# AIBluefisher/DAGSfM

Hardware: AMD Instinct MI355X
Metric: verified image-pairs/sec (+ RANSAC hypotheses/sec) at 4096 feats/image (higher is better)
Workload: dtype u8 matching (int8 MFMA) + f64 verification

## Files before the change

### dagsfm_amd/csrc/match_kernels.hip

```cpp
#include <hip/hip_runtime.h>
#include <stdint.h>

#include <type_traits>

#include "kernels.h"

typedef int v4i __attribute__((ext_vector_type(4)));
typedef int v16i __attribute__((ext_vector_type(16)));

template <int B, int E, typename F>
__device__ __forceinline__ void static_for(F&& f) {
  if constexpr (B < E) {
    f(std::integral_constant<int, B>());
    static_for<B + 1, E>(f);
  }
}

__global__ __launch_bounds__(256) void k0_prepare(const uint8_t* __restrict__ in_u8,
                                                  int8_t* __restrict__ out_s8,
                                                  int32_t* __restrict__ rterm,
                                                  uint64_t n_rows) {
  const uint64_t gid = (uint64_t)blockIdx.x * blockDim.x + threadIdx.x;
  const uint64_t row = gid >> 3;
  const uint32_t chunk = (uint32_t)gid & 7u;
  if (row >= n_rows) return;
  const uint4 v = reinterpret_cast<const uint4*>(in_u8)[row * 8 + chunk];
  uint32_t w[4] = {v.x, v.y, v.z, v.w};
  int32_t sum = 0;
#pragma unroll
  for (int k = 0; k < 4; ++k) {
    sum += (int32_t)((w[k] & 0xffu) + ((w[k] >> 8) & 0xffu) + ((w[k] >> 16) & 0xffu) + (w[k] >> 24));
    w[k] ^= 0x80808080u;
  }
  uint4 o;
  o.x = w[0]; o.y = w[1]; o.z = w[2]; o.w = w[3];
  reinterpret_cast<uint4*>(out_s8)[row * 8 + chunk] = o;
  sum += __shfl_xor(sum, 1);
  sum += __shfl_xor(sum, 2);
  sum += __shfl_xor(sum, 4);
  if (chunk == 0) rterm[row] = 128 * (sum - 16384);
}

template <int Q>
__device__ __forceinline__ void k1_epilogue_quarter(const v16i& a, int& best, int& second, int& t, int& btile, int tile) {
  if constexpr (Q == 0) {
    asm volatile(
        "v_max3_i32 %[t], %[a0], %[a1], %[a2]\n\t"
        "v_max3_i32 %[t], %[t], %[a3], %[a4]\n\t"
        "v_max3_i32 %[t], %[t], %[a5], %[a6]"
        : [t] "=&v"(t)
        : [a0] "v"(a[0]), [a1] "v"(a[1]), [a2] "v"(a[2]), [a3] "v"(a[3]), [a4] "v"(a[4]), [a5] "v"(a[5]), [a6] "v"(a[6]));
  } else if constexpr (Q == 1) {
    asm volatile(
        "v_max3_i32 %[t], %[t], %[a0], %[a1]\n\t"
        "v_max3_i32 %[t], %[t], %[a2], %[a3]\n\t"
        "v_max3_i32 %[t], %[t], %[a4], %[a5]"
        : [t] "+v"(t)
        : [a0] "v"(a[7]), [a1] "v"(a[8]), [a2] "v"(a[9]), [a3] "v"(a[10]), [a4] "v"(a[11]), [a5] "v"(a[12]));
  } else if constexpr (Q == 2) {
    asm volatile(
        "v_max3_i32 %[t], %[t], %[a0], %[a1]\n\t"
        "v_max3_i32 %[t], %[t], %[a2], %[s]\n\t"
        "v_min_i32 %[s], %[t], %[b]"
        : [t] "+v"(t), [s] "+v"(second)
        : [b] "v"(best), [a0] "v"(a[13]), [a1] "v"(a[14]), [a2] "v"(a[15]));
  } else {
    asm volatile(
        "v_cmp_gt_i32 vcc, %[t], %[b]\n\t"
        "v_cndmask_b32 %[bt], %[bt], %[tile], vcc\n\t"
        "v_max_i32 %[b], %[t], %[b]"
        : [b] "+v"(best), [bt] "+v"(btile)
        : [t] "v"(t), [tile] "v"(tile)
        : "vcc");
  }
}

#ifndef K1_LDS_DMA
#define K1_LDS_DMA 0
#endif
__device__ __forceinline__ int lds_off(int col, int chunk) {
  return col * 128 + ((chunk ^ ((col >> 1) & 7)) << 4);
}

template <bool GATHER>
__global__ __launch_bounds__(256, 2) void k1_best_rows(const K1Params p) {
  const uint32_t d = p.order ? p.order[blockIdx.x] : blockIdx.x;
  const uint32_t rb = blockIdx.y;
  const uint2 ab = p.dpairs[d];
  const uint32_t a_rows = GATHER ? p.e_cnt[d] : p.img_rows[ab.x];
  if (rb * 512u >= a_rows) return;
  const uint32_t b_cols = p.img_rows[ab.y];
  const uint32_t a_row0 = (GATHER ? 0u : p.img_row0[ab.x]) + rb * 512u;
  const uint32_t b_row0 = p.img_row0[ab.y];

  const int tid = threadIdx.x;
  const int lane = tid & 63;
  const int wave = tid >> 6;
  const int l31 = lane & 31;
  const int half = lane >> 5;
  const bool active = rb * 512u + (uint32_t)wave * 128u < a_rows;

  __shared__ __attribute__((aligned(16))) int8_t sB[2][64 * 128];
  __shared__ __attribute__((aligned(16))) int sC[2][64];

  v4i afrag[4][4];
  int rterm_i[4];
  bool valid[4];
  {
    const uint2* ent = GATHER ? p.entries + p.e_off[d] : nullptr;
    const uint32_t img0 = GATHER ? p.img_row0[ab.x] : 0u;
#pragma unroll
    for (int rt = 0; rt < 4; ++rt) {
      const uint32_t r = a_row0 + wave * 128 + rt * 32 + l31;
      valid[rt] = GATHER ? (r < a_rows) : active;
      uint32_t grow = r;
      if (GATHER) grow = valid[rt] ? img0 + ent[r].y : 0u;
      const int8_t* arow = p.desc + (size_t)grow * 128;
#pragma unroll
      for (int ks = 0; ks < 4; ++ks) {
        const v4i z = {0, 0, 0, 0};
        afrag[rt][ks] = valid[rt] ? *reinterpret_cast<const v4i*>(arow + ks * 32 + half * 16) : z;
      }
      rterm_i[rt] = valid[rt] ? p.rterm[grow] : 0;
    }
  }
  int best[4], second[4], btile[4];
#pragma unroll
  for (int rt = 0; rt < 4; ++rt) {
    best[rt] = -rterm_i[rt];
    second[rt] = -rterm_i[rt];
    btile[rt] = 0;
  }

  const int8_t* bimg = p.desc + (size_t)b_row0 * 128;
  const int32_t* rt_b = p.rterm + b_row0;
  const uint32_t nsteps = b_cols >> 6;

  int cstage = 0;
#if K1_LDS_DMA
  const int wave_u = __builtin_amdgcn_readfirstlane(wave);
  int src_off[2];
#pragma unroll
  for (int u = 0; u < 2; ++u) {
    const int L = tid + 256 * u;
    src_off[u] = ((L & ~7) | ((L & 7) ^ ((L >> 4) & 7))) * 16;
  }
  auto stage_tile = [&](const int8_t* src, int buf) {
#pragma unroll
    for (int u = 0; u < 2; ++u)
      __builtin_amdgcn_global_load_lds((const __attribute__((address_space(1))) void*)(src + src_off[u]),
                                       (__attribute__((address_space(3))) void*)(&sB[buf][(wave_u * 64 + 256 * u) * 16]), 16, 0, 0);
  };
  stage_tile(bimg, 0);
  cstage = rt_b[tid & 63];
  if (tid < 64) sC[0][tid] = cstage + (1 << 21);
  __syncthreads();
#else
  v4i stage[2];
#pragma unroll
  for (int u = 0; u < 2; ++u) stage[u] = *reinterpret_cast<const v4i*>(bimg + (size_t)(tid + 256 * u) * 16);
  cstage = rt_b[tid & 63];
#pragma unroll
  for (int u = 0; u < 2; ++u) {
    const int q = tid + 256 * u;
    *reinterpret_cast<v4i*>(&sB[0][lds_off(q >> 3, q & 7)]) = stage[u];
  }
  if (tid < 64) sC[0][tid] = cstage + (1 << 21);
  __syncthreads();
#endif
  asm volatile("s_waitcnt vmcnt(0)" ::: "memory");

  for (uint32_t s = 0; s < nsteps; ++s) {
    const int cur = s & 1;
    const bool more = (s + 1) < nsteps;
    if (more) {
      const int8_t* src = bimg + (size_t)(s + 1) * 64 * 128;
#if K1_LDS_DMA
      stage_tile(src, cur ^ 1);
#else
#pragma unroll
      for (int u = 0; u < 2; ++u) stage[u] = *reinterpret_cast<const v4i*>(src + (size_t)(tid + 256 * u) * 16);
#endif
      cstage = rt_b[(s + 1) * 64 + (tid & 63)];
    }
    if (active) {
      v4i bf0[4], bf1[4];
#pragma unroll
      for (int ks = 0; ks < 4; ++ks) {
        bf0[ks] = *reinterpret_cast<const v4i*>(&sB[cur][lds_off(l31, ks * 2 + half)]);
        bf1[ks] = *reinterpret_cast<const v4i*>(&sB[cur][lds_off(32 + l31, ks * 2 + half)]);
      }
      v16i ci0, ci1;
#pragma unroll
      for (int q = 0; q < 4; ++q) {
        const v4i c0 = *reinterpret_cast<const v4i*>(&sC[cur][8 * q + 4 * half]);
        const v4i c1 = *reinterpret_cast<const v4i*>(&sC[cur][32 + 8 * q + 4 * half]);
#pragma unroll
        for (int e = 0; e < 4; ++e) {
          ci0[4 * q + e] = c0[e];
          ci1[4 * q + e] = c1[e];
        }
      }
      v16i acc[3];
      int tmax;
      int tile_v[2];
      asm volatile("v_mov_b32 %0, %2\n\tv_mov_b32 %1, %3" : "=&v"(tile_v[0]), "=v"(tile_v[1]) : "s"(2 * s), "s"(2 * s + 1));
#define K1_MFMA(K, KS)                                                                                 \
  acc[(K) % 3] = __builtin_amdgcn_mfma_i32_32x32x32_i8(((K) >> 2) ? bf1[KS] : bf0[KS], afrag[(K)&3][KS], \
                                                       (KS) == 0 ? (((K) >> 2) ? ci1 : ci0) : acc[(K) % 3], 0, 0, 0)
#define K1_EPI(E)                                                                                        \
  {                                                                                                      \
    constexpr int ek = (E) >> 2, eq = (E)&3, ert = ek & 3;                                               \
    k1_epilogue_quarter<eq>(acc[ek % 3], best[ert], second[ert], tmax, btile[ert], tile_v[ek >> 2]);          \
  }
      static_for<0, 4>([&](auto KS) { K1_MFMA(0, KS.value); });
      __builtin_amdgcn_sched_barrier(0);
      static_for<0, 28>([&](auto J) {
        constexpr int j = J.value;
        K1_MFMA((j >> 2) + 1, j & 3);
        __builtin_amdgcn_sched_barrier(0);
        if constexpr (j >= 1) {
          K1_EPI(j - 1);
          __builtin_amdgcn_sched_barrier(0);
        }
      });
      static_for<27, 32>([&](auto E) { K1_EPI(E.value); });
      __builtin_amdgcn_sched_barrier(0);
#undef K1_MFMA
#undef K1_EPI
    }
    if (more) {
#if !K1_LDS_DMA
#pragma unroll
      for (int u = 0; u < 2; ++u) {
        const int q = tid + 256 * u;
        *reinterpret_cast<v4i*>(&sB[cur ^ 1][lds_off(q >> 3, q & 7)]) = stage[u];
      }
#endif
      if (tid < 64) sC[cur ^ 1][tid] = cstage + (1 << 21);
    }
    __syncthreads();
  }

  if (!active) return;
  const uint64_t out0 = (GATHER ? p.e_off[d] : p.d_out_off[d]) + rb * 512u + wave * 128;
  int32_t* out = p.out + out0;
  int32_t* out_s = p.out_s + out0;
#pragma unroll
  for (int rt = 0; rt < 4; ++rt) {
    const int oB = __shfl_xor(best[rt], 32);
    const int oS = __shfl_xor(second[rt], 32);
    const int oT = __shfl_xor(btile[rt], 32);
    const int B = max(best[rt], oB);
    const int S = max(min(best[rt], oB), max(second[rt], oS));
    const bool take = (oB > best[rt]) || (oB == best[rt] && oT < btile[rt]);
    const bool both = oB == best[rt] && oT == btile[rt];
    const int T = take ? oT : btile[rt];
    const int set = both ? 2 : ((take ? 1 : 0) ^ half);
    const int best_dot = B + rterm_i[rt];
    const int second_dot = S + rterm_i[rt];
    int res = -1;
    if (best_dot > 0) {
      const float bn = p.lut[min(best_dot, 262144)];
      if (!(bn > p.max_distance)) {
        const float sn = p.lut[min(second_dot, 262144)];
        const float rhs = __fmul_rn(p.max_ratio, sn);
        if (!(bn >= rhs)) res = T * 4 + set;
      }
    }
    if (half == (rt & 1) && valid[rt]) {
      out[rt * 32 + l31] = res;
      if (res >= 0) out_s[rt * 32 + l31] = second_dot;
    }
  }
}

template <bool GATHER>
__global__ __launch_bounds__(256) void k1_resolve_index(const K1Params p) {
  const uint32_t d = blockIdx.x;
  const uint2 ab = p.dpairs[d];
  const uint32_t a_rows = GATHER ? p.e_cnt[d] : p.img_rows[ab.x];
  const int tid = threadIdx.x;
  const int lane = tid & 63, wave = tid >> 6;
  const uint32_t b_row0 = p.img_row0[ab.y];
  const uint32_t a_img0 = p.img_row0[ab.x];
  const int8_t* bimg = p.desc + (size_t)b_row0 * 128;
  const int32_t* rt_b = p.rterm + b_row0;
  const uint2* ent = GATHER ? p.entries + p.e_off[d] : nullptr;
  const int g = lane >> 3;
  for (uint32_t row_w = wave * 64u; row_w < a_rows; row_w += 256u) {
    const uint64_t o0 = (GATHER ? p.e_off[d] : p.d_out_off[d]) + row_w;
    int32_t* out = p.out + o0;
    const int32_t* out_s = p.out_s + o0;
    const bool in_range = !GATHER || row_w + (uint32_t)lane < a_rows;
    const int t = in_range ? out[lane] : -1;
    const int s_appr = t >= 0 ? out_s[lane] : 0;
    const uint32_t my_row = GATHER ? (in_range ? ent[row_w + lane].y : 0u) : row_w + (uint32_t)lane;
    unsigned long long mask = __ballot(t >= 0);
    constexpr int RU = 4;
    while (mask) {
      int r_l[RU], tile_l[RU], set_l[RU], sap_l[RU];
      uint32_t grow_l[RU];
      bool on[RU];
#pragma unroll
      for (int u = 0; u < RU; ++u) {
        on[u] = mask != 0ull;
        const int r = on[u] ? (__ffsll((long long)mask) - 1) : 0;
        if (on[u]) mask &= mask - 1;
        r_l[u] = r;
        const int code = on[u] ? __builtin_amdgcn_readlane(t, r) : 0;
        tile_l[u] = code >> 2;
        set_l[u] = code & 3;
        sap_l[u] = __builtin_amdgcn_readlane(s_appr, r);
        grow_l[u] = a_img0 + (uint32_t)__builtin_amdgcn_readlane((int)my_row, r);
      }
      v4i x[RU], y[RU][4];
      int ct[RU][4], col[RU][4], rti[RU];
#pragma unroll
      for (int u = 0; u < RU; ++u) {
        x[u] = *reinterpret_cast<const v4i*>(p.desc + (size_t)grow_l[u] * 128 + (lane & 7) * 16);
        rti[u] = p.rterm[grow_l[u]];
        const bool both = set_l[u] == 2;
#pragma unroll
        for (int i = 0; i < 4; ++i) {
          col[u][i] = both ? i * 8 + g : 8 * (2 * (i & 1) + (g >> 2)) + 4 * set_l[u] + (g & 3);
          if (i < 2 || both) {
            const int c = tile_l[u] * 32 + col[u][i];
            y[u][i] = *reinterpret_cast<const v4i*>(bimg + (size_t)c * 128 + (lane & 7) * 16);
            ct[u][i] = rt_b[c];
          }
        }
      }
#pragma unroll
      for (int u = 0; u < RU; ++u) {
        const bool both = set_l[u] == 2;
        int k1 = INT32_MIN, k2 = INT32_MIN;
#pragma unroll
        for (int i = 0; i < 4; ++i) {
          if (i < 2 || both) {
            int acc = 0;
#pragma unroll
            for (int e = 0; e < 4; ++e) acc = __builtin_amdgcn_sdot4(x[u][e], y[u][i][e], acc, false);
            acc += __shfl_xor(acc, 1);
            acc += __shfl_xor(acc, 2);
            acc += __shfl_xor(acc, 4);
            const int key = (int)((uint32_t)(acc + ct[u][i]) << 5) | (31 - col[u][i]);
            k2 = max(k2, min(k1, key));
            k1 = max(k1, key);
          }
        }
#pragma unroll
        for (int o = 8; o < 64; o <<= 1) {
          const int o1 = __shfl_xor(k1, o), o2 = __shfl_xor(k2, o);
          k2 = max(min(k1, o1), max(k2, o2));
          k1 = max(k1, o1);
        }
        if (lane == 0 && on[u]) {
          const int bias = rti[u] + (1 << 21);
          const int best_dot = (k1 >> 5) + bias;
          const int second_dot = max(sap_l[u], (k2 >> 5) + bias);
          const float bn = p.lut[min(best_dot, 262144)];
          const float sn = p.lut[min(second_dot, 262144)];
          const float rhs = __fmul_rn(p.max_ratio, sn);
          out[r_l[u]] = (bn >= rhs) ? -1 : tile_l[u] * 32 + (31 - (k1 & 31));
        }
      }
    }
  }
}

#ifdef DSM_CHECK_BUILD
__global__ __launch_bounds__(256) void k1_best_rows_dot4(const K1Params p) {
  const uint32_t d = p.order ? p.order[blockIdx.x] : blockIdx.x;
  const uint32_t rb = blockIdx.y;
  const uint2 ab = p.dpairs[d];
  const uint32_t a_rows = p.img_rows[ab.x];
  if (rb * 512u >= a_rows) return;
  const uint32_t b_cols = p.img_rows[ab.y];
  const uint32_t a_row0 = p.img_row0[ab.x], b_row0 = p.img_row0[ab.y];
  const int tid = threadIdx.x;
  const uint32_t row[2] = {rb * 512u + tid, rb * 512u + 256u + tid};
  const bool has2 = row[1] < a_rows;
  __shared__ __attribute__((aligned(16))) int8_t sB[2][64 * 128];
  __shared__ int sR[2][64];
  v4i a[2][8];
  int rterm_i[2];
#pragma unroll
  for (int r = 0; r < 2; ++r) {
    const uint32_t rr = (r == 0 || has2) ? row[r] : row[0];
    const int8_t* arow = p.desc + (size_t)(a_row0 + rr) * 128;
#pragma unroll
    for (int c = 0; c < 8; ++c) a[r][c] = *reinterpret_cast<const v4i*>(arow + c * 16);
    rterm_i[r] = p.rterm[a_row0 + rr];
  }
  int best[2] = {0, 0}, second[2] = {0, 0}, best_j[2] = {-1, -1};
  const uint32_t nsteps = b_cols >> 6;
  v4i st[2];
  int sr = 0;
  auto fetch = [&](uint32_t s) {
#pragma unroll
    for (int u = 0; u < 2; ++u)
      st[u] = *reinterpret_cast<const v4i*>(p.desc + (size_t)(b_row0 + s * 64) * 128 + (size_t)(tid + 256 * u) * 16);
    sr = p.rterm[b_row0 + s * 64 + (tid & 63)];
  };
  auto commit = [&](int buf) {
#pragma unroll
    for (int u = 0; u < 2; ++u) *reinterpret_cast<v4i*>(&sB[buf][(tid + 256 * u) * 16]) = st[u];
    if (tid < 64) sR[buf][tid] = sr;
  };
  fetch(0);
  commit(0);
  __syncthreads();
  for (uint32_t s = 0; s < nsteps; ++s) {
    const int cur = s & 1;
    const bool more = s + 1 < nsteps;
    if (more) fetch(s + 1);
    for (int j = 0; j < 64; ++j) {
      int acc[2] = {0, 0};
#pragma unroll
      for (int c = 0; c < 8; ++c) {
        const v4i b = *reinterpret_cast<const v4i*>(&sB[cur][j * 128 + c * 16]);
#pragma unroll
        for (int e = 0; e < 4; ++e) {
          acc[0] = __builtin_amdgcn_sdot4(a[0][c][e], b[e], acc[0], false);
          acc[1] = __builtin_amdgcn_sdot4(a[1][c][e], b[e], acc[1], false);
        }
      }
      const int cterm = sR[cur][j] + (1 << 21);
#pragma unroll
      for (int r = 0; r < 2; ++r) {
        const int dist = acc[r] + rterm_i[r] + cterm;
        if (dist > best[r]) {
          second[r] = best[r];
          best[r] = dist;
          best_j[r] = (int)(s * 64 + j);
        } else if (dist > second[r]) {
          second[r] = dist;
        }
      }
    }
    if (more) commit(cur ^ 1);
    __syncthreads();
  }
#pragma unroll
  for (int r = 0; r < 2; ++r) {
    if (r == 1 && !has2) break;
    int res = -1;
    if (best_j[r] >= 0) {
      const float bn = p.lut[min(best[r], 262144)];
      if (!(bn > p.max_distance)) {
        const float sn = p.lut[min(second[r], 262144)];
        const float rhs = __fmul_rn(p.max_ratio, sn);
        if (!(bn >= rhs)) res = best_j[r];
      }
    }
    p.out[p.d_out_off[d] + row[r]] = res;
  }
}

#endif

__device__ __forceinline__ bool guided_filter(int mode, const float* M, float x1, float y1, float x2, float y2,
                                              float max_residual) {
  if (mode == 1) {
    const float Fx1_0 = (M[0] * x1 + M[1] * y1) + M[2];
    const float Fx1_1 = (M[3] * x1 + M[4] * y1) + M[5];
    const float Fx1_2 = (M[6] * x1 + M[7] * y1) + M[8];
    const float Ftx2_0 = (M[0] * x2 + M[3] * y2) + M[6];
    const float Ftx2_1 = (M[1] * x2 + M[4] * y2) + M[7];
    const float x2tFx1 = (x2 * Fx1_0 + y2 * Fx1_1) + Fx1_2;
    return x2tFx1 * x2tFx1 / (((Fx1_0 * Fx1_0 + Fx1_1 * Fx1_1) + Ftx2_0 * Ftx2_0) + Ftx2_1 * Ftx2_1) > max_residual;
  }
  const float Hp_0 = (M[0] * x1 + M[1] * y1) + M[2];
  const float Hp_1 = (M[3] * x1 + M[4] * y1) + M[5];
  const float Hp_2 = (M[6] * x1 + M[7] * y1) + M[8];
  const float d0 = Hp_0 / Hp_2 - x2, d1 = Hp_1 / Hp_2 - y2;
  return d0 * d0 + d1 * d1 > max_residual;
}

__global__ __launch_bounds__(256) void kg_best_rows(const KgParams p) {
  const uint32_t d = blockIdx.x;
  const uint32_t rb = blockIdx.y;
  const uint2 ab = p.dpairs[d];
  const uint32_t a_rows = p.img_rows[ab.x];
  if (rb * 256u >= a_rows) return;
  const uint32_t b_cols = p.img_rows[ab.y];
  const uint32_t a_feat = p.img_nfeat[ab.x], b_feat = p.img_nfeat[ab.y];
  const uint32_t a_row0 = p.img_row0[ab.x], b_row0 = p.img_row0[ab.y];
  const int tid = threadIdx.x;
  const uint32_t row = rb * 256u + tid;

  __shared__ __attribute__((aligned(16))) int8_t sB[64 * 128];
  __shared__ int sR[64];
  __shared__ float sX[64], sY[64];

  const float* gp = p.gparams + (size_t)d * 12;
  float M[9];
#pragma unroll
  for (int k = 0; k < 9; ++k) M[k] = gp[k];
  const int mode = (int)gp[9];
  const bool swap = gp[10] != 0.0f;

  v4i a[8];
  const int8_t* arow = p.desc + (size_t)(a_row0 + row) * 128;
#pragma unroll
  for (int c = 0; c < 8; ++c) a[c] = *reinterpret_cast<const v4i*>(arow + c * 16);
  const int rterm_i = p.rterm[a_row0 + row];
  float xr = 0.0f, yr = 0.0f;
  if (row < a_feat) {
    xr = (float)p.kp[(size_t)(a_row0 + row) * 2];
    yr = (float)p.kp[(size_t)(a_row0 + row) * 2 + 1];
  }
  int best = 0, second = 0, best_j = -1;
  for (uint32_t j0 = 0; j0 < b_cols; j0 += 64) {
    __syncthreads();
#pragma unroll
    for (int u = 0; u < 2; ++u) {
      const int q = tid + 256 * u;
      *reinterpret_cast<v4i*>(&sB[q * 16]) = *reinterpret_cast<const v4i*>(p.desc + (size_t)(b_row0 + j0) * 128 + (size_t)q * 16);
    }
    if (tid < 64) {
      const uint32_t col = j0 + tid;
      sR[tid] = p.rterm[b_row0 + col];
      const bool real = col < b_feat;
      sX[tid] = real ? (float)p.kp[(size_t)(b_row0 + col) * 2] : 0.0f;
      sY[tid] = real ? (float)p.kp[(size_t)(b_row0 + col) * 2 + 1] : 0.0f;
    }
    __syncthreads();
    for (int j = 0; j < 64; ++j) {
      int acc = 0;
#pragma unroll
      for (int c = 0; c < 8; ++c) {
        const v4i b = *reinterpret_cast<const v4i*>(&sB[j * 128 + c * 16]);
#pragma unroll
        for (int e = 0; e < 4; ++e) acc = __builtin_amdgcn_sdot4(a[c][e], b[e], acc, false);
      }
      int dist = acc + rterm_i + sR[j] + (1 << 21);
      const float xc = sX[j], yc = sY[j];
      const bool filtered = swap ? guided_filter(mode, M, xc, yc, xr, yr, p.max_residual)
                                 : guided_filter(mode, M, xr, yr, xc, yc, p.max_residual);
      if (filtered) dist = 0;
      if (dist > best) {
        second = best;
        best = dist;
        best_j = (int)(j0 + j);
      } else if (dist > second) {
        second = dist;
      }
    }
  }
  int res = -1;
  if (best_j >= 0) {
    const float bn = p.lut[min(best, 262144)];
    if (!(bn > p.max_distance)) {
      const float sn = p.lut[min(second, 262144)];
      const float rhs = __fmul_rn(p.max_ratio, sn);
      if (!(bn >= rhs)) res = best_j;
    }
  }
  if (row < a_rows) p.out[p.d_out_off[d] + row] = res;
}

template <bool WRITE>
__global__ __launch_bounds__(256) void k2_cross_compact(const K2Params p) {
  const uint32_t pi = blockIdx.x;
  const uint4 pd = p.pair_dir[pi];
  const int32_t* m12 = p.m + p.d_out_off[pd.x];
  const int32_t* m21 = p.cross_check ? (p.m + p.d_out_off[pd.y]) : nullptr;
  const uint32_t n1 = pd.z;
  const int tid = threadIdx.x;
  const int lane = tid & 63, wave = tid >> 6;
  __shared__ uint32_t wsum[4];
  uint32_t running = 0;
  uint2* dst = nullptr;
  if (WRITE) dst = reinterpret_cast<uint2*>(p.matches) + p.offsets[pi];
  for (uint32_t base = 0; base < n1; base += 256) {
    const uint32_t i = base + tid;
    int j = -1;
    bool ok = false;
    if (i < n1) {
      j = m12[i];
      ok = j >= 0;
      if (ok && p.cross_check) ok = (m21[j] == (int32_t)i);
    }
    const unsigned long long bal = __ballot(ok);
    const uint32_t before = __popcll(bal & ((1ull << lane) - 1ull));
    if (lane == 0) wsum[wave] = __popcll(bal);
    __syncthreads();
    uint32_t wbase = 0, total = 0;
#pragma unroll
    for (int w = 0; w < 4; ++w) {
      const uint32_t c = wsum[w];
      if (w < wave) wbase += c;
      total += c;
    }
    if (WRITE && ok) dst[running + wbase + before] = make_uint2(i, (uint32_t)j);
    running += total;
    __syncthreads();
  }
  if (!WRITE && tid == 0) p.counts[pi] = running;
}

template <bool WRITE>
__global__ __launch_bounds__(256) void k2_entries_compact(const K2eParams p) {
  const uint32_t pi = blockIdx.x;
  const uint32_t n = p.e_cnt[pi];
  const uint2* ent = p.entries + p.e_off[pi];
  const int32_t* m21 = p.out2 + p.e_off[pi];
  const int tid = threadIdx.x;
  const int lane = tid & 63, wave = tid >> 6;
  __shared__ uint32_t wsum[4];
  uint32_t running = 0;
  uint2* dst = nullptr;
  if (WRITE) dst = reinterpret_cast<uint2*>(p.matches) + p.offsets[pi];
  for (uint32_t base = 0; base < n; base += 256) {
    const uint32_t k = base + tid;
    uint2 e = make_uint2(0, 0);
    bool ok = false;
    if (k < n) {
      e = ent[k];
      ok = m21[k] == (int32_t)e.x;
    }
    const unsigned long long bal = __ballot(ok);
    const uint32_t before = __popcll(bal & ((1ull << lane) - 1ull));
    if (lane == 0) wsum[wave] = __popcll(bal);
    __syncthreads();
    uint32_t wbase = 0, total = 0;
#pragma unroll
    for (int w = 0; w < 4; ++w) {
      const uint32_t c = wsum[w];
      if (w < wave) wbase += c;
      total += c;
    }
    if (WRITE && ok) dst[running + wbase + before] = e;
    running += total;
    __syncthreads();
  }
  if (!WRITE && tid == 0) p.counts[pi] = running;
}

__global__ __launch_bounds__(1024) void k_scan_counts(const uint32_t* __restrict__ counts,
                                                      uint64_t* __restrict__ offsets, uint32_t n,
                                                      uint64_t* __restrict__ running_total) {
  __shared__ uint64_t wsum[16];
  __shared__ uint64_t carry;
  const int tid = threadIdx.x, lane = tid & 63, wave = tid >> 6;
  if (tid == 0) carry = *running_total;
  __syncthreads();
  for (uint32_t base = 0; base < n; base += 1024) {
    const uint32_t i = base + tid;
    const uint64_t v = i < n ? counts[i] : 0;
    uint64_t x = v;
#pragma unroll
    for (int o = 1; o < 64; o <<= 1) {
      const uint64_t y = __shfl_up(x, o);
      if (lane >= o) x += y;
    }
    if (lane == 63) wsum[wave] = x;
    __syncthreads();
    uint64_t wbase = 0, total = 0;
#pragma unroll
    for (int w = 0; w < 16; ++w) {
      if (w < wave) wbase += wsum[w];
      total += wsum[w];
    }
    if (i < n) offsets[i] = carry + wbase + x - v;
    __syncthreads();
    if (tid == 0) carry += total;
    __syncthreads();
  }
  if (tid == 0) {
    offsets[n] = carry;
    *running_total = carry;
  }
}

void launch_k0(const uint8_t* in_u8, int8_t* out_s8, int32_t* rterm, uint64_t n_rows, hipStream_t st) {
  if (n_rows == 0) return;
  const uint64_t threads = n_rows * 8;
  const uint32_t blocks = (uint32_t)((threads + 255) / 256);
  hipLaunchKernelGGL(k0_prepare, dim3(blocks), dim3(256), 0, st, in_u8, out_s8, rterm, n_rows);
}

void launch_k1(const K1Params& p, uint32_t n_directed, uint32_t max_row_blocks, hipStream_t st) {
  if (n_directed == 0 || max_row_blocks == 0) return;
  if (p.entries)
    hipLaunchKernelGGL(k1_best_rows<true>, dim3(n_directed, (max_row_blocks + 1) / 2), dim3(256), 0, st, p);
  else
    hipLaunchKernelGGL(k1_best_rows<false>, dim3(n_directed, (max_row_blocks + 1) / 2), dim3(256), 0, st, p);
}
#ifdef DSM_CHECK_BUILD
void launch_k1_dot4(const K1Params& p, uint32_t n_directed, uint32_t max_row_blocks, hipStream_t st) {
  if (n_directed == 0 || max_row_blocks == 0) return;
  hipLaunchKernelGGL(k1_best_rows_dot4, dim3(n_directed, (max_row_blocks + 1) / 2), dim3(256), 0, st, p);
}
#endif
void launch_k1_resolve(const K1Params& p, uint32_t n_directed, uint32_t max_row_blocks, hipStream_t st) {
  if (n_directed == 0 || max_row_blocks == 0) return;
  if (p.entries)
    hipLaunchKernelGGL(k1_resolve_index<true>, dim3(n_directed), dim3(256), 0, st, p);
  else
    hipLaunchKernelGGL(k1_resolve_index<false>, dim3(n_directed), dim3(256), 0, st, p);
}
void launch_k2_entries(const K2eParams& p, uint32_t n_pairs, bool write, hipStream_t st) {
  if (n_pairs == 0) return;
  if (write)
    hipLaunchKernelGGL(k2_entries_compact<true>, dim3(n_pairs), dim3(256), 0, st, p);
  else
    hipLaunchKernelGGL(k2_entries_compact<false>, dim3(n_pairs), dim3(256), 0, st, p);
}

void launch_kg(const KgParams& p, uint32_t n_directed, uint32_t max_row_blocks, hipStream_t st) {
  if (n_directed == 0 || max_row_blocks == 0) return;
  hipLaunchKernelGGL(kg_best_rows, dim3(n_directed, max_row_blocks), dim3(256), 0, st, p);
}

struct GuidedPlan {
  uint64_t src_off, dst_off;
  uint32_t count, from_guided;
};
__global__ __launch_bounds__(64) void k_guided_assemble(const GuidedPlan* plan, const uint32_t* old_inl, const uint32_t* guided,
                                                        uint32_t* dst, uint32_t n_pairs) {
  for (uint32_t pi = blockIdx.x; pi < n_pairs; pi += gridDim.x) {
    const GuidedPlan pl = plan[pi];
    const uint2* s = reinterpret_cast<const uint2*>(pl.from_guided ? guided : old_inl) + pl.src_off;
    uint2* d = reinterpret_cast<uint2*>(dst) + pl.dst_off;
    for (uint32_t i = threadIdx.x; i < pl.count; i += 64) d[i] = s[i];
  }
}
void launch_guided_assemble(const void* plan, const uint32_t* old_inl, const uint32_t* guided, uint32_t* dst, uint32_t n_pairs,
                            hipStream_t st) {
  if (!n_pairs) return;
  hipLaunchKernelGGL(k_guided_assemble, dim3(n_pairs < 8192 ? n_pairs : 8192), dim3(64), 0, st,
                     static_cast<const GuidedPlan*>(plan), old_inl, guided, dst, n_pairs);
}

void launch_k2(const K2Params& p, uint32_t n_pairs, bool write, hipStream_t st) {
  if (n_pairs == 0) return;
  if (write)
    hipLaunchKernelGGL(k2_cross_compact<true>, dim3(n_pairs), dim3(256), 0, st, p);
  else
    hipLaunchKernelGGL(k2_cross_compact<false>, dim3(n_pairs), dim3(256), 0, st, p);
}

void launch_scan(const uint32_t* counts, uint64_t* offsets, uint32_t n, uint64_t* running_total, hipStream_t st) {
  hipLaunchKernelGGL(k_scan_counts, dim3(1), dim3(1024), 0, st, counts, offsets, n, running_total);
}
```

Baseline: 272,600.

## Balance gathered row fragments across waves and skip empty MFMA fragments

In the gather variant of the best-rows kernel, the 32-row fragments of a block are now spread evenly across the four waves instead of assigning a fixed 128 rows per wave. Each wave runs an MFMA/epilogue schedule specialised at compile time for its actual fragment count (1 to 4). This avoids issuing matrix multiplies for padded, invalid rows when a block holds fewer than 512 gathered entries. It costs extra code size from four unrolled schedule variants and a runtime branch that picks one.

```diff
diff --git a/dagsfm_amd/csrc/match_kernels.hip b/dagsfm_amd/csrc/match_kernels.hip
--- a/dagsfm_amd/csrc/match_kernels.hip
+++ b/dagsfm_amd/csrc/match_kernels.hip
@@ -98,7 +98,15 @@
   const int wave = tid >> 6;
   const int l31 = lane & 31;
   const int half = lane >> 5;
-  const bool active = rb * 512u + (uint32_t)wave * 128u < a_rows;
+  uint32_t frag0 = (uint32_t)wave * 4u;
+  int nf_w = 4;
+  if constexpr (GATHER) {
+    const uint32_t nf = (min(512u, a_rows - rb * 512u) + 31u) >> 5;
+    const uint32_t w = (uint32_t)__builtin_amdgcn_readfirstlane(wave);
+    frag0 = w * (nf >> 2) + min(w, nf & 3u);
+    nf_w = (int)((nf >> 2) + (w < (nf & 3u) ? 1u : 0u));
+  }
+  const bool active = GATHER ? nf_w > 0 : rb * 512u + (uint32_t)wave * 128u < a_rows;
 
   __shared__ __attribute__((aligned(16))) int8_t sB[2][64 * 128];
   __shared__ __attribute__((aligned(16))) int sC[2][64];
@@ -111,8 +119,8 @@
     const uint32_t img0 = GATHER ? p.img_row0[ab.x] : 0u;
 #pragma unroll
     for (int rt = 0; rt < 4; ++rt) {
-      const uint32_t r = a_row0 + wave * 128 + rt * 32 + l31;
-      valid[rt] = GATHER ? (r < a_rows) : active;
+      const uint32_t r = a_row0 + (frag0 + rt) * 32 + l31;
+      valid[rt] = GATHER ? (rt < nf_w && r < a_rows) : active;
       uint32_t grow = r;
       if (GATHER) grow = valid[rt] ? img0 + ent[r].y : 0u;
       const int8_t* arow = p.desc + (size_t)grow * 128;
@@ -205,27 +213,31 @@
       int tmax;
       int tile_v[2];
       asm volatile("v_mov_b32 %0, %2\n\tv_mov_b32 %1, %3" : "=&v"(tile_v[0]), "=v"(tile_v[1]) : "s"(2 * s), "s"(2 * s + 1));
-#define K1_MFMA(K, KS)                                                                                 \
-  acc[(K) % 3] = __builtin_amdgcn_mfma_i32_32x32x32_i8(((K) >> 2) ? bf1[KS] : bf0[KS], afrag[(K)&3][KS], \
-                                                       (KS) == 0 ? (((K) >> 2) ? ci1 : ci0) : acc[(K) % 3], 0, 0, 0)
+#define K1_MFMA(K, KS)                                                                                        \
+  acc[(K) % 3] = __builtin_amdgcn_mfma_i32_32x32x32_i8(((K) / NF) ? bf1[KS] : bf0[KS], afrag[(K) % NF][KS],    \
+                                                       (KS) == 0 ? (((K) / NF) ? ci1 : ci0) : acc[(K) % 3], 0, 0, 0)
 #define K1_EPI(E)                                                                                        \
   {                                                                                                      \
-    constexpr int ek = (E) >> 2, eq = (E)&3, ert = ek & 3;                                               \
-    k1_epilogue_quarter<eq>(acc[ek % 3], best[ert], second[ert], tmax, btile[ert], tile_v[ek >> 2]);          \
-  }
-      static_for<0, 4>([&](auto KS) { K1_MFMA(0, KS.value); });
-      __builtin_amdgcn_sched_barrier(0);
-      static_for<0, 28>([&](auto J) {
-        constexpr int j = J.value;
-        K1_MFMA((j >> 2) + 1, j & 3);
+    constexpr int ek = (E) >> 2, eq = (E)&3, ert = ek % NF;                                              \
+    k1_epilogue_quarter<eq>(acc[ek % 3], best[ert], second[ert], tmax, btile[ert], tile_v[ek / NF]);     \
+  }
+      static_for<(GATHER ? 1 : 4), 5>([&](auto NFc) {
+        constexpr int NF = NFc.value;
+        if (GATHER && nf_w != NF) return;
+        static_for<0, 4>([&](auto KS) { K1_MFMA(0, KS.value); });
         __builtin_amdgcn_sched_barrier(0);
-        if constexpr (j >= 1) {
-          K1_EPI(j - 1);
+        static_for<0, 8 * NF - 4>([&](auto J) {
+          constexpr int j = J.value;
+          K1_MFMA((j >> 2) + 1, j & 3);
           __builtin_amdgcn_sched_barrier(0);
-        }
+          if constexpr (j >= 1) {
+            K1_EPI(j - 1);
+            __builtin_amdgcn_sched_barrier(0);
+          }
+        });
+        static_for<8 * NF - 5, 8 * NF>([&](auto E) { K1_EPI(E.value); });
+        __builtin_amdgcn_sched_barrier(0);
       });
-      static_for<27, 32>([&](auto E) { K1_EPI(E.value); });
-      __builtin_amdgcn_sched_barrier(0);
 #undef K1_MFMA
 #undef K1_EPI
     }
@@ -243,7 +255,7 @@
   }
 
   if (!active) return;
-  const uint64_t out0 = (GATHER ? p.e_off[d] : p.d_out_off[d]) + rb * 512u + wave * 128;
+  const uint64_t out0 = (GATHER ? p.e_off[d] : p.d_out_off[d]) + rb * 512u + frag0 * 32u;
   int32_t* out = p.out + out0;
   int32_t* out_s = p.out_s + out0;
 #pragma unroll
```

Measured after the change: 273,200 (median of 6 runs). Within noise of the previous version (+0.2%).
